# ethereum/pos-evolution

Hardware: AMD Instinct MI355X
Metric: attestations aggregated/sec + get_head() p50 latency at 1M validators (higher is better)
Workload: dtype int32

## Files before the change

include/posevo_profile.h:

```cpp
#ifndef POSEVO_PROFILE_H
#define POSEVO_PROFILE_H
#include "posevo.h"
#ifdef __cplusplus
extern "C" {
#endif

#define PE_KERNEL_G1_ACCUMULATE 0
#define PE_KERNEL_G1_NORMALISE  1
#define PE_KERNEL_VOTES         2
#define PE_KERNEL_TREE          3
#define PE_KERNEL_LMD           4
#define PE_KERNEL_PARTICIPATION 5
#define PE_KERNEL_BITS_UNION    6
#define PE_KERNEL_G2_ACCUMULATE 7
#define PE_KERNEL_G2_NORMALISE  8
#define PE_KERNEL_G1_TREE       9
#define PE_KERNEL_ATT_GROUP     10
#define PE_KERNEL_ATT_VALIDATE  11
#define PE_KERNEL_PAIR_INGEST_VALIDATE 12
#define PE_KERNEL_PAIR_PLAN_LMD        13
#define PE_KERNEL_PAIR_MEMBERS_VOTES   14
#define PE_KERNEL_PAIR_UNION_TREE      15
#define PE_KERNEL_G2_DECOMPRESS 16
#define PE_KERNEL_COUNT         17
int pe_profile_enable(pe_engine* h, int on);
int pe_profile_reset(pe_engine* h);
int pe_profile_get(pe_engine* h, int kernel, uint64_t* launches, double* total_ms);
int pe_profile_timeline(pe_engine* h, int32_t* kernel, double* start_ms, double* duration_ms, uint32_t cap, uint32_t* out_n);

int pe_profile_queue_classes(pe_engine* h, int32_t out_class[4]);
int pe_profile_arena_growths(const pe_engine* h, uint64_t* out);
int pe_profile_committee_sums(const pe_engine* h, uint32_t* out_tables_with_sums, uint32_t* out_groups_by_complement);
int pe_profile_accumulate_mhz(pe_engine* h, double* out_mhz, uint32_t cap, uint32_t* out_n);
int pe_profile_pairing_gt(pe_engine* h, const uint8_t* g1_points96, const uint8_t* g2_points192, uint64_t n_pairs,
                          const uint32_t* offsets, uint32_t n_groups, uint8_t* out576);
#define PE_BATCH_CHUNK_MAX 64
int pe_profile_batch_set_chunk(pe_engine* h, uint32_t chunk);
int pe_profile_batch_stats(const pe_engine* h, uint32_t out[8]);
int pe_profile_batch_gt(const pe_engine* h, uint8_t* out576);

#define PE_VERIFY_STRIPE_MAX 16
int pe_profile_verify_set_stripe(pe_engine* h, uint32_t k);
int pe_profile_verify_stats(const pe_engine* h, uint32_t out[5]);
int pe_profile_verify_sums(const pe_engine* h, uint32_t n_groups, uint8_t* out_pk96, uint8_t* out_sig192);

#define PE_VERIFY_RESIDENT_STATS 11
int pe_profile_verify_resident_stats(const pe_engine* h, uint32_t out[PE_VERIFY_RESIDENT_STATS]);

#ifdef __cplusplus
}
#endif
#endif
```

pos_evolution_amd/_abi.py:

```python
from __future__ import annotations

import ctypes as C
import os

_HERE = os.path.dirname(os.path.abspath(__file__))
LIB_PATH = os.environ.get("POSEVO_LIB_PATH") or os.path.join(_HERE, "libposevo.so")

PE_OK = 0
PE_ERR_NO_DEVICE = -2
PE_ERR_UNKNOWN_PARENT = -4
PE_ERR_UNKNOWN_ROOT = -9
PE_ERR_CAPACITY = -10
PE_ERR_STATE = -14
PE_ERR_TIMEOUT = -15
PE_DIST_SINGLE_COMM = 1
PE_SIG_G2_COMPRESSED, PE_SIG_G2_UNCOMPRESSED, PE_SIG_CHECK_SUBGROUP = 1, 2, 0x100
PE_SIG_STATUS_IDENTITY = 4
PE_BLS_INVALID, PE_BLS_VALID, PE_BLS_BAD_POINT, PE_BLS_UNDECIDED = 0, 1, 2, 3
PE_VERIFY_APPLY = 0x1
PE_VERIFY_RESIDENT_STATS = 11
NONE32 = 0xFFFFFFFF

PE_VAL_ACTIVE, PE_VAL_SLASHED, PE_VAL_EQUIVOCATING, PE_VAL_ACTIVE_PREV = 0x01, 0x02, 0x04, 0x08
PE_ATT_FLAG_SIGNATURE_VALID, PE_ATT_FLAG_FROM_BLOCK = 0x1, 0x2
PE_G1_PARTIAL_BYTES = 192
PE_EXCHANGE_EXTRA = 512
PE_DIST_ID_BYTES = 256
(PE_KERNEL_G1_ACCUMULATE, PE_KERNEL_G1_NORMALISE, PE_KERNEL_VOTES, PE_KERNEL_TREE, PE_KERNEL_LMD,
 PE_KERNEL_PARTICIPATION, PE_KERNEL_BITS_UNION, PE_KERNEL_G2_ACCUMULATE, PE_KERNEL_G2_NORMALISE,
 PE_KERNEL_G1_TREE, PE_KERNEL_ATT_GROUP, PE_KERNEL_ATT_VALIDATE, PE_KERNEL_PAIR_INGEST_VALIDATE,
 PE_KERNEL_PAIR_PLAN_LMD, PE_KERNEL_PAIR_MEMBERS_VOTES, PE_KERNEL_PAIR_UNION_TREE, PE_KERNEL_G2_DECOMPRESS,
 PE_KERNEL_COUNT) = range(18)
KERNEL_NAMES = ["g1_accumulate", "g1_normalise", "votes", "tree", "lmd", "participation", "bits_union",
                "g2_accumulate", "g2_normalise", "g1_tree", "att_group", "att_validate", "pair_ingest_validate",
                "pair_plan_lmd", "pair_members_votes", "pair_union_tree", "g2_decompress"]

ATT_STATUS_NAMES = {
    0: "ok", 1: "target epoch not current or previous", 2: "target epoch != epoch(slot)",
    3: "unknown target root", 4: "unknown beacon block root", 5: "block after attestation slot",
    6: "target not ancestor of beacon block", 7: "attestation slot not in the past", 8: "no committee table",
    9: "committee index out of range", 10: "bits length mismatch", 11: "empty or invalid indices",
    12: "bad signature", 13: "outside inclusion window", 14: "source mismatch",
    32: "slasher: target epoch in the future", 33: "slasher: target epoch left the window",
    34: "slasher: data table of the epoch is full",
}
PE_ATT_UNKNOWN_TARGET_ROOT, PE_ATT_UNKNOWN_BEACON_BLOCK_ROOT = 3, 4
PE_SLASH_FUTURE_TARGET, PE_SLASH_TOO_OLD, PE_SLASH_TABLE_FULL = 32, 33, 34
PE_SLASH_APPLY = 1
PE_SLASH_DOUBLE, PE_SLASH_SURROUND = 1, 2


class pe_config(C.Structure):
    _fields_ = [
        ("slots_per_epoch", C.c_uint64), ("seconds_per_slot", C.c_uint64), ("intervals_per_slot", C.c_uint64),
        ("safe_slots_to_update_justified", C.c_uint64), ("proposer_score_boost", C.c_uint64),
        ("effective_balance_increment", C.c_uint64), ("min_attestation_inclusion_delay", C.c_uint64),
        ("max_validators_per_committee", C.c_uint64), ("filter_slashed", C.c_uint32), ("device", C.c_int32),
        ("reserve_validators", C.c_uint64), ("reserve_blocks", C.c_uint32), ("max_committee_tables", C.c_uint32),
        ("vote_expiry_slots", C.c_uint64),
    ]


class pe_attestation(C.Structure):
    _fields_ = [
        ("slot", C.c_uint64), ("index", C.c_uint64), ("beacon_block_root", C.c_uint8 * 32),
        ("source_epoch", C.c_uint64), ("source_root", C.c_uint8 * 32),
        ("target_epoch", C.c_uint64), ("target_root", C.c_uint8 * 32),
        ("bits_offset", C.c_uint32), ("n_bits", C.c_uint32), ("flags", C.c_uint32), ("reserved0", C.c_uint32),
    ]


assert C.sizeof(pe_attestation) == 144


class pe_state_ctx(C.Structure):
    _fields_ = [
        ("slot", C.c_uint64), ("chain_tip_root", C.c_uint8 * 32),
        ("current_justified_epoch", C.c_uint64), ("current_justified_root", C.c_uint8 * 32),
        ("previous_justified_epoch", C.c_uint64), ("previous_justified_root", C.c_uint8 * 32),
        ("base_reward_per_increment", C.c_uint64),
    ]


class pe_prune_stats(C.Structure):
    _fields_ = [("blocks_before", C.c_uint32), ("blocks_after", C.c_uint32), ("votes_remapped", C.c_uint64),
                ("votes_orphaned", C.c_uint64)]


# ... 221 lines not shown
```

pos_evolution_amd/csrc/att_bodies.inc:

```
#include <algorithm>
#include "att_rules.h"
#include "kernels.h"
#include "wave64.h"

namespace posevo {

namespace {

constexpr uint32_t VAL_EQUIVOCATING_BIT = 0x04u;
constexpr uint32_t ERR_INVALID_ARG = 1, ERR_CAPACITY = 10, ERR_NO_COMMITTEES = 11;

struct Row9 { uint4 q[9]; };
__device__ __forceinline__ void load_row(Row9& r, const uint4* __restrict__ rows, uint32_t i)
{
    const uint4* p = rows + (size_t)9 * i;
#pragma unroll
    for (int k = 0; k < 9; ++k) r.q[k] = p[k];
}
__device__ __forceinline__ unsigned long long u64_of(uint32_t lo, uint32_t hi) { return ((unsigned long long)hi << 32) | lo; }
__device__ __forceinline__ unsigned long long row_slot(const Row9& r) { return u64_of(r.q[0].x, r.q[0].y); }
__device__ __forceinline__ unsigned long long row_index(const Row9& r) { return u64_of(r.q[0].z, r.q[0].w); }
__device__ __forceinline__ unsigned long long row_source_epoch(const Row9& r) { return u64_of(r.q[3].x, r.q[3].y); }
__device__ __forceinline__ unsigned long long row_target_epoch(const Row9& r) { return u64_of(r.q[5].z, r.q[5].w); }

// ... 424 lines not shown
    }
}
struct Root2 { uint4 lo, hi; };
struct BlockStoreDev {
    const BlockTableDev& bt;
    __device__ __forceinline__ uint32_t find(const Root2& r) const { return find_block_dev(bt, r.lo, r.hi); }
    __device__ __forceinline__ uint32_t handle(uint32_t idx) const { return bt.pos_of_idx[idx]; }
    __device__ __forceinline__ unsigned long long slot_of(uint32_t idx) const { return bt.slot_pos[bt.pos_of_idx[idx]]; }
    __device__ __forceinline__ uint32_t ancestor(uint32_t idx, unsigned long long slot) const
    {
        uint32_t p = bt.pos_of_idx[idx];
        while (bt.slot_pos[p] > slot && bt.parent_pos[p] != NONE32) p = bt.parent_pos[p];
        return p;
    }
};
}

namespace {
__device__ __forceinline__ void att_validate_fc_body(const uint32_t g , const ValidateFcArgs& a)
{
    const uint4* __restrict__ rows = static_cast<const uint4*>(a.rows);
    const AttGroup* __restrict__ grp = a.grp;
    const AttPlan* __restrict__ plan = a.plan;
    const uint32_t cap = a.cap;
    const BlockTableDev& bt = a.bt;
    const FcCtx& fc = a.fc;
    const uint32_t* __restrict__ union_info = a.union_info;
    AttRow* __restrict__ out_rows = a.out_rows;
    int32_t* __restrict__ status_dev = a.status_dev;
    int32_t* __restrict__ status_host = a.status_host;
    uint32_t* __restrict__ count_host = a.count_host;
    uint32_t* __restrict__ err_host = a.err_host;
    const uint32_t ng = plan->n_groups;
    if (ng > cap) {
        if (g < ng) status_dev[g] = -1;
        if (g == 0) *err_host = ERR_CAPACITY;
        return;
    }
    if (g >= ng) return;
    const AttGroup G = grp[g];
    Row9 r;
    load_row(r, rows, G.rep);
    const unsigned long long slot = row_slot(r), tep = row_target_epoch(r), spe = fc.slots_per_epoch;
    const FcVerdict v = att_fork_choice_status(BlockStoreDev{bt}, (r.q[8].z & FLAG_FROM_BLOCK) != 0, slot, tep, Root2{r.q[6], r.q[7]},
                                               Root2{r.q[1], r.q[2]}, fc.cur_slot, fc.cur_epoch, fc.prev_epoch, spe);
    int32_t st = v.status;
    if (st == ST_OK) st = (int32_t)G.status_agg;
    const uint32_t cnt = union_info[2 * g], overlap = union_info[2 * g + 1];
    if (st == ST_OK) st = att_indexed_status(G.sig_valid != 0, overlap != 0, cnt);
    out_rows[g] = att_row_fork_choice(G.member_base, G.size, G.out_word, v.block, tep, slot, g, g);
    status_dev[g] = st;
    status_host[g] = st;
    if (count_host) count_host[g] = st == ST_OK ? cnt : 0u;
}
}

namespace {
__device__ __forceinline__ void lmd_vm_tables_body(const unsigned long long v , const LmdVmArgs& a)
{
    const AttRow* __restrict__ rows = a.rows;
    const TablesDev& tables = a.tables;
    const uint32_t* __restrict__ cs0 = a.crow_start[0];
    const uint32_t* __restrict__ cs1 = a.crow_start[1];
    const uint32_t* __restrict__ cl0 = a.crow_list[0];
    const uint32_t* __restrict__ cl1 = a.crow_list[1];
    const AttPlan* __restrict__ plan = a.plan;
    const uint32_t* __restrict__ bit_arena = a.bit_arena;
    const uint8_t* __restrict__ flags = a.flags;
    unsigned long long* __restrict__ vote_key = reinterpret_cast<unsigned long long*>(a.vote_key);
    uint32_t* __restrict__ vote_block = a.vote_block;
    uint32_t* __restrict__ vote_slot = a.vote_slot;
    const uint32_t* __restrict__ gates = a.gates;
    if (v >= a.n_val) return;
    uint32_t best_e = 0, best_order = NONE32, new_block = NONE32, new_slot = 0;
    bool loaded = false;
    for (int t = 0; t < 2; ++t) {
        if (!tables.t[t].valid || plan->n_rows_table[t] == 0) continue;
        const uint32_t c = tables.t[t].inv_comm[v];
        if (c == NONE32) continue;
        const uint32_t* crow_start = t ? cs1 : cs0;
        const uint32_t* crow_list = t ? cl1 : cl0;
        const uint32_t kb = crow_start[c], ke = crow_start[c + 1];
        if (kb == ke) continue;
        if (!loaded) {
            if (flags[v] & VAL_EQUIVOCATING_BIT) return;
            best_e = (uint32_t)(vote_key[v] >> 32);
            loaded = true;
        }
        const uint32_t i = tables.t[t].inv_pos[v];
        for (uint32_t k = kb; k < ke; ++k) {
            const AttRow r = rows[crow_list[k]];
            if (i >= r.n_bits) continue;
            if (gates[r.gate] != 0) continue;
            if (!((bit_arena[r.bits_word + (i >> 5)] >> (i & 31)) & 1u)) continue;
            if (r.epoch_p1 > best_e || (r.epoch_p1 == best_e && new_block != NONE32 && r.order < best_order)) {
                best_e = r.epoch_p1;
                best_order = r.order;
                new_block = r.block_idx;
                new_slot = r.slot;
            }
        }
    }
    if (new_block != NONE32) {
        vote_key[v] = ((unsigned long long)best_e << 32) | 0xFFFFFFFFull;
        vote_block[v] = new_block;
        if (vote_slot) vote_slot[v] = new_slot;
    }
}
}

}
```

pos_evolution_amd/csrc/engine_g1.cpp:

```cpp
#include "engine_internal.h"

using namespace posevo;

namespace posevo {

void g1_stream_guard(pe_engine* h, hipStream_t s)
{
    if (h->side_ever && s != h->side_stream && s != h->fin_stream && s != h->norm_stream) (void)hipStreamWaitEvent(s, h->ev_join, 0);
}

int build_points30(pe_engine* h, uint64_t n)
{
    HIP_TRY(h, h->d_points30.ensure(std::max<size_t>(128, 4ull * G1_ROW_WORDS * n)));
    launch_g1_table_s30(h->stream, h->d_points.as<uint32_t>(), h->d_points30.as<uint32_t>(), n);
    HIP_TRY(h, hipGetLastError());
    h->points30_valid = true;
    return PE_OK;
}

int launch_g1_planned(pe_engine* h, const uint32_t* d_points, const uint32_t* d_members, const uint32_t* d_bits,
                      const G1Group* d_groups, const G1Plan& plan, uint8_t* d_out96, uint32_t* dev_jac,
                      hipStream_t s, hipStream_t fin, DevBuf* partials, DevBuf* lane_partials, const AttPlan* plan_dev,
                      const uint32_t* d_members1, uint64_t caller_rows, const G1Complement* cm)
{
    if (plan.n_groups == 0) return PE_OK;
    if (!s) s = h->stream;
    if (!fin) fin = s;
    if (!partials) partials = &h->d_partials;
    if (!lane_partials) lane_partials = &h->d_lane_partials;
    PE_TRY(ensure_quiesced(h, *partials,
                           std::max<size_t>(PE_G1_PARTIAL_BYTES, (size_t)PE_G1_PARTIAL_BYTES * plan.n_partials)));
    const size_t lane_bytes = (size_t)G1_LANE_PARTIAL_BYTES * G1_WG * ((plan.n_slots + G1_WG - 1) / G1_WG);
    PE_TRY(ensure_quiesced(h, *lane_partials, std::max<size_t>(PE_G1_PARTIAL_BYTES, lane_bytes)));
    const uint32_t* d_points30;
    if (d_points == h->d_points.as<uint32_t>()) {
        if (!h->points30_valid) return fail(h, PE_ERR_STATE, "the registry's table of the accumulation's field form was not built");
        d_points30 = h->d_points30.as<uint32_t>();
    } else {
        const uint64_t n_rows = caller_rows;
        if (d_points != h->d_tmp_points.as<uint32_t>() || 4ull * G1_ROW_WORDS * n_rows > h->d_tmp_points.cap)
            return fail(h, PE_ERR_STATE, "G1 sum over an unknown point table");
        HIP_TRY(h, h->d_tmp_points30.ensure(std::max<size_t>(128, 4ull * G1_ROW_WORDS * n_rows)));
        launch_g1_table_s30(s, d_points, h->d_tmp_points30.as<uint32_t>(), n_rows);
        d_points30 = h->d_tmp_points30.as<uint32_t>();
    }
    const bool chain = fin != s && fin == h->fin_stream;
    const int exclusive = chain && h->tune.exclusive && h->blocks.size() <= 4096 ? 1 : 0;
    const uint32_t sparse_max = cm && cm->info ? h->tune.g1_sparse_max() : 0u;
    const uint32_t* sparse_info = sparse_max ? cm->info : nullptr;
    if (sparse_max)
        launch_g1_absentees(s, d_points30, d_members, d_members1, d_bits, d_groups, plan.n_groups, plan_dev, cm->cmpl, sparse_info,
                            sparse_max, partials->as<uint32_t>());
    {
        const bool skip = !h->prof_timeline && s != h->stream && (h->acc_launches++ & 3) != 0;
        ProfScope ps(h, PE_KERNEL_G1_ACCUMULATE, s, skip);
        unsigned long long* clock_rec = nullptr;
        if (h->profiling) {
            if (!h->acc_clock && hipHostMalloc(reinterpret_cast<void**>(&h->acc_clock), 16ull * pe_engine::ACC_CLOCK_RING,
                                               hipHostMallocDefault) != hipSuccess) {
                (void)hipGetLastError();
                h->acc_clock = nullptr;
            }
            if (h->acc_clock) {
                clock_rec = h->acc_clock + 2 * (h->acc_clock_n++ % pe_engine::ACC_CLOCK_RING);
                clock_rec[0] = clock_rec[1] = 0;
            }
        }
        launch_g1_accumulate(s, d_points30, d_members, d_bits, d_groups, plan.n_groups, plan.n_slots,
                             lane_partials->as<uint32_t>(), partials->as<uint32_t>(), plan_dev, d_members1, exclusive, clock_rec,
                             cm ? cm->cmpl : nullptr, sparse_info, sparse_max);
    }
    hipStream_t ts = fin;
    if (ts != s) {
        HIP_TRY(h, hipEventRecord(h->ev_acc, s));
        HIP_TRY(h, hipStreamWaitEvent(ts, h->ev_acc, 0));
    }
    {
        ProfScope ps(h, PE_KERNEL_G1_TREE, ts);
        launch_g1_tree(ts, lane_partials->as<uint32_t>(), d_groups, plan.n_groups, plan.n_slots, partials->as<uint32_t>(),
                       ts != s ? 1 : 0,
                       plan_dev, exclusive, sparse_max ? cm->cmpl : nullptr, sparse_info, sparse_max);
    }
    hipStream_t ns = fin;
    if (chain && h->norm_stream) {
        ns = h->norm_stream;
        HIP_TRY(h, hipEventRecord(h->ev_tree, ts));
        HIP_TRY(h, hipStreamWaitEvent(ns, h->ev_tree, 0));
    } else if (ts != fin) {
        HIP_TRY(h, hipEventRecord(h->ev_tree, ts));
        HIP_TRY(h, hipStreamWaitEvent(fin, h->ev_tree, 0));
    }
    if (cm)
        for (int t = 0; t < 2; ++t)
            if (cm->ev[t]) HIP_TRY(h, hipStreamWaitEvent(ns, cm->ev[t], 0));
    {
        ProfScope ps(h, PE_KERNEL_G1_NORMALISE, ns);
        launch_g1_finish(ns, partials->as<uint32_t>(), d_groups, plan.n_groups, 0, 0, d_out96, dev_jac, plan_dev,
                         cm ? cm->cmpl : nullptr, cm ? cm->sums[0] : nullptr, cm ? cm->sums[1] : nullptr);
    }
    HIP_TRY(h, hipGetLastError());
    return PE_OK;
}

void committee_sums_drop(pe_engine* h)
{
// ... 690 lines not shown
```

pos_evolution_amd/csrc/engine_internal.h:

```cpp
#pragma once
#include <hip/hip_runtime.h>
#include <dlfcn.h>
#include <rccl/rccl.h>

#include <algorithm>
#include <array>
#include <chrono>
#include <cstdlib>
#include <map>
#include <cstdio>
#include <cstddef>
#include <cstring>
#include <functional>
#include <memory>
#include <new>
#include <numeric>
#include <string>
#include <thread>
#include <unordered_map>
#include <vector>

#include "../../include/posevo.h"
#include "../../include/posevo_profile.h"
#include "att_rules.h"
// ... 223 lines not shown
    DevBuf d_vote_slot;
    DevBuf d_sbalance, d_sflags;
    bool state_view_set = false;
    std::vector<uint8_t> h_flags;
    DevBuf d_activation_epoch, d_exit_epoch;
    bool epochs_set = false;
    DevBuf d_active, d_active_wg;
    bool active_valid = false;
    uint64_t active_epoch = 0;
    uint32_t active_n = 0;
    hipEvent_t ev_active_read = nullptr;
    bool active_read_pending = false;
    DevBuf d_rbalance, d_inactivity, d_withdrawable;
    bool balances_set = false;
    DevBuf d_registry_wg;
    DevBuf d_pubkey_leaf, d_withdrawal_credentials, d_activation_eligibility;
    bool static_set = false;
    DevBuf d_ssz_zero;
    bool ssz_zero_ready = false;
    DevBuf d_ssz_validator_roots;
    DevBuf d_ssz_level[2];
    DevBuf d_ssz_chunks;
    DevBuf d_bls;
    struct ResidentVerify {
        bool valid = false;
        uint64_t rr_generation = 0, res_generation = 0;
        int arena = 0;
        uint32_t n_in = 0;
        bool checked_subgroup = false;
    } rv;
    uint32_t* keep_pk = nullptr;
    std::vector<uint8_t> verify_head;
    uint32_t verify_resident_stats[PE_VERIFY_RESIDENT_STATS] = {};
    DevBuf d_batch;
    uint32_t batch_chunk = 2;
    uint32_t batch_stats[8] = {};
    uint8_t batch_gt[576] = {};
    DevBuf d_verify;
    uint32_t verify_stripe = 16;
    uint32_t verify_stats[5] = {};
    std::vector<uint8_t> verify_sums_pk, verify_sums_sig;

    bool tree_dirty = true;
    DevBuf d_tsize, d_tparent, d_trank, d_tleaf, d_tpos, d_tidx, d_direct, d_weights, d_totals, d_head;
    DevBuf d_broot_tab, d_broots, d_bslot_pos;
    uint32_t broot_mask = 0;
    std::vector<uint32_t> h_pos_of_idx;
    PinBuf h_head;
    uint32_t votes_grid = 0;
    bool weights_stale = false;

    std::vector<CommitteeTable> tables;
    uint64_t table_stamp = 0;
    size_t last_table = 0;

    DevBuf d_partials, d_lane_partials, d_out96, d_tmp_points, d_tmp_be;

    struct PipeArena {
        DevBuf d_stage, d_outblk;
        PinBuf h_stage, h_pin;
        DevBuf d_res_bits, d_res_info;
        DevBuf d_partials, d_lane_partials;
        DevBuf d_rr_tab, d_rr;
        DevBuf d_sig_in, d_sig_pts, d_sig_status;
        DevBuf d_res_points;
        uint32_t rr_rows_cap = 0, rr_comm_cap = 0, rr_tab_size = 0;
        DevBuf x_rr_tab, x_rr, x_res_bits, x_res_info;
        uint32_t x_rows_cap = 0, x_comm_cap = 0, x_tab_size = 0;
        DevBuf d_xsend, d_xrecv, d_xrows, d_xbits, d_xn;
        size_t stage_cursor = 0, out_cursor = 0;
        uint64_t table_stamp_at_begin = 0;
        uint64_t generation = 0;
        std::vector<std::function<int()>> pending;
        hipEvent_t ev_main = nullptr, ev_side = nullptr, ev_aux = nullptr;
        hipEvent_t ev_leg = nullptr;
        bool leg_used = false;
        bool fenced = false, side_used = false, aux_used = false;
        bool fence_pending = false;
        bool aux_reads_scratch = false;
    };
    static constexpr int MAX_ARENAS = 16;
    int n_arenas = 3;
    PipeArena arena[MAX_ARENAS];
    int cur = 0;
    PipeArena& A() { return arena[cur]; }
    bool pipelining = false;
    uint64_t pipes_begun = 0, pipes_completed = 0;
    hipStream_t side_stream = nullptr;
    uint64_t arena_growths = 0;
    bool queues_distinct = false;
    hipStream_t fin_stream = nullptr;
    hipStream_t norm_stream = nullptr;
    hipEvent_t ev_tree = nullptr;
    hipStream_t g1_tail() const { return norm_stream ? norm_stream : fin_stream; }
    hipStream_t aux_stream = nullptr;
    hipStream_t aux_owned = nullptr;
    hipStream_t prep_stream = nullptr;
    DevBuf d_shuffle_scratch;
    hipStream_t sums_stream = nullptr;
    DevBuf d_sum_groups, d_sum_lane;
    uint32_t last_cmpl_groups = 0;
    hipEvent_t ev_aux_fork = nullptr;
    hipEvent_t ev_aux_switch = nullptr;
    static constexpr uint32_t STATE_ON_SIDE_MAX_ROWS = 1024;
    bool aux_busy = false;
    bool state_work_on_main = false;
    hipEvent_t ev_acc = nullptr;
    struct SigSeg {
        int arena;
        uint32_t n;
        bool compressed, check_subgroup;
        bool streaming;
        const uint8_t* d_in;
        const uint8_t* copy_from;
        size_t bytes;
        uint32_t* d_pts; int32_t* d_status;
        const UnionGroup* d_ug; const uint32_t* d_member_row; uint32_t ng_bound; const AttPlan* plan_dev;
        uint8_t* o_sig; uint32_t* o_bad; int32_t* o_st;
        uint32_t* keep_mont48; uint32_t* keep_bad;
    };
    std::vector<SigSeg> sig_batch;
    hipEvent_t ev_sig = nullptr;
    hipEvent_t ev_fork = nullptr, ev_join = nullptr;
    bool side_busy = false;
    bool side_ever = false;
    bool streaming = false;
    std::vector<std::function<int()>> deferred;
    struct HeldFc {
        bool active = false;
        int arena = -1;
        bool have_fc = false;
        bool have_head = false;
        ValidateFcArgs validate{};
        LmdVmArgs lmd{};
        VotesArgs votes{};
        TreeArgs tree{};
        std::function<int()> between;
        std::vector<std::function<int()>> g1;
        bool fence_pending = false;
    } held;
    bool pairing = std::getenv("POSEVO_PAIR") == nullptr || std::atoi(std::getenv("POSEVO_PAIR")) != 0;
    struct Tune {
        static int env(const char* name, int dflt)
        {
            const char* e = std::getenv(name);
            return e && *e ? std::atoi(e) : dflt;
        }
        int exclusive = env("POSEVO_ACC_EXCLUSIVE", 1);
        int state_on = env("POSEVO_STATE_ON", 2);
        int sig_batch = env("POSEVO_SIG_BATCH", 8);
        int queue_probe = env("POSEVO_QUEUE_PROBE", 1);
        int committee_sums = env("POSEVO_COMMITTEE_SUMS", 1);
        int g1_sparse = env("POSEVO_G1_SPARSE", 1);
        uint32_t g1_sparse_max() const
        {
            return g1_sparse <= 0 ? 0u : g1_sparse == 1 ? G1_SPARSE_MAX : std::min<uint32_t>((uint32_t)g1_sparse, G1_SPARSE_CAP);
        }
        uint32_t ssz_tile_log2 = (uint32_t)std::min<int>(SSZ_TILE_LOG2, std::max<int>(SSZ_TILE_LOG2_MIN, env("POSEVO_SSZ_TILE_LOG2", SSZ_TILE_LOG2)));
    } tune;

    struct ResGroup { uint32_t byte_off, n_bits, word, sig_valid, tag; };
    std::vector<ResGroup> res_groups;
    std::shared_ptr<std::vector<uint32_t>> res_info_host;
    bool res_valid = false;
    int res_arena = 0;
    uint64_t res_generation = 0;

    struct ResidentRows {
        bool valid = false;
        int arena = 0;
        uint32_t n_in = 0;
        const void* rows = nullptr;
        TablesDev tables{};
        uint64_t generation = 0;
        int set = 0;
        uint32_t n_groups = 0;
    } rr;

    int g1_tune_calls = 0;
    float g1_tune_best[2] = {1e30f, 1e30f};
    uint32_t g1_target_slots = 0;
    hipEvent_t g1_tune_ev[2] = {nullptr, nullptr};
    bool points30_valid = false;
    DevBuf d_points30, d_tmp_points30;

    ncclComm_t comm = nullptr, comm_g1 = nullptr;
    int early_rc = PE_OK;
    uint32_t xchg_blocks = 0;
    uint64_t xchg_nval = 0;
    bool last_agg_on_side = false;
    int dist_rank = 0, dist_world = 1;
    DevBuf d_xchg, d_xpart, d_xgather;
    pe_collectives coll{};
    bool coll_custom = false;
    bool dist_single_comm = false;
    bool dist_wedged = false;
    uint32_t dist_timeout_ms = 30000;
    uint32_t dist_max_groups = 0;
    hipEvent_t ev_xchg = nullptr;
    bool dist_ready() const { return comm != nullptr || coll_custom; }

    struct Slasher {
        bool enabled = false;
        uint32_t history = 0, max_data = 0;
        uint64_t n_val = 0;
        bool have_window = false;
        uint64_t window = 0;
        DevBuf d_rec, d_ids, d_counter, d_evidence;
        struct EpochData {
            std::vector<std::array<uint8_t, 128>> data;
// ... 2 lines not shown
        std::vector<EpochData> epochs;
        bool on_device = false;
        uint32_t tab_size = 0;
        DevBuf d_data, d_count, d_tab;
        DevBuf d_work;
        std::vector<uint32_t> dev_count;
    } slasher;

    bool profiling = false;
    uint64_t acc_launches = 0;
    static constexpr uint32_t ACC_CLOCK_RING = 4096;
    unsigned long long* acc_clock = nullptr;
    uint64_t acc_clock_n = 0;
    KernelProfile prof[PE_KERNEL_COUNT];
    bool prof_timeline = false;
    bool prof_dominant_only = false;
    hipEvent_t prof_base = nullptr;
    struct TimelineEntry { int32_t kernel; float start_ms, dur_ms; };
    std::vector<TimelineEntry> prof_tl;
    std::vector<hipEvent_t> event_pool;
    HostTrace trace;
};

namespace posevo {

int fail(pe_engine* h, int code, const std::string& msg);
int hip_fail(pe_engine* h, hipError_t e, const char* what);
#define HIP_TRY(h, expr)                                        \
    do {                                                        \
        hipError_t _e = (expr);                                 \
        if (_e != hipSuccess) return hip_fail((h), _e, #expr);  \
    } while (0)
#define PE_TRY(expr)              \
    do {                          \
        const int _rc = (expr);   \
        if (_rc) return _rc;      \
    } while (0)

struct ProfScope {
    pe_engine* h;
    int k;
    hipStream_t s;
    hipEvent_t a = nullptr, b = nullptr;
    static hipEvent_t take(pe_engine* h)
    {
        if (!h->event_pool.empty()) { hipEvent_t e = h->event_pool.back(); h->event_pool.pop_back(); return e; }
        hipEvent_t e = nullptr;
        return hipEventCreate(&e) == hipSuccess ? e : nullptr;
    }
    ProfScope(pe_engine* h_, int k_, hipStream_t s_ = nullptr, bool sampled_out = false) : h(h_), k(k_), s(s_ ? s_ : h_->stream)
    {
        if (!h->profiling || sampled_out) return;
        if (h->prof_dominant_only && k != PE_KERNEL_G1_ACCUMULATE) return;
        if ((k == PE_KERNEL_ATT_GROUP || k == PE_KERNEL_ATT_VALIDATE) && !h->prof_timeline) return;
        a = take(h);
        b = take(h);
        if (!a || !b) { a = b = nullptr; return; }
        (void)hipEventRecord(a, s);
    }
    ~ProfScope()
    {
        if (!a) return;
        (void)hipEventRecord(b, s);
        h->prof[k].pending.emplace_back(a, b);
    }
};

int run_deferred(pe_engine* h);
int complete_arena(pe_engine* h, int ai);
void complete_oldest_if_ready(pe_engine* h);
int flush_pending(pe_engine* h);
int enter(pe_engine* h);
extern const uint8_t NEG_G1_BE96[96];
int draw_scalars(pe_engine* h, std::vector<uint64_t>& out);
int pairing_run(pe_engine* h, const char* who, const uint8_t* g1, const uint8_t* g2, uint64_t n_pairs, const uint32_t* offsets,
                uint32_t n_groups, int32_t* verdict, uint8_t* out576);
using WireAt = std::function<const uint8_t*(uint32_t)>;
int verify_pairs_run(pe_engine* h, const char* who, uint32_t n, const WireAt& pk_at, const WireAt& msg_at, const WireAt& sig_at,
                     int32_t* verdict);
struct ResPoints { uint32_t *pk_xyzz48, *sig_mont48, *sig_bad; size_t bytes; };
inline ResPoints res_points_layout(void* base, uint32_t n)
{
    const size_t rows = std::max<uint32_t>(n, 1);
    Layout l;
    const auto pk = l.take<uint32_t>(48 * rows), sig = l.take<uint32_t>(48 * rows), bad = l.take<uint32_t>(rows);
    return ResPoints{pk.at(base), sig.at(base), bad.at(base), l.total()};
}
inline int refuse_dist(pe_engine* h, const char* who)
{
    return fail(h, PE_ERR_STATE, std::string(who) + ": the handle exchanges with other ranks (pe_dist_init); "
                                                    "the sharded handles are not supported");
}
int need_init(pe_engine* h, bool flush = true, bool keep_held = false);
bool hold_eligible(const pe_engine* h);
int held_issue(pe_engine* h);
int launch_rows_paired(pe_engine* h, const IngestArgs& ia, const AttPlanArgs& pa, const MembersArgs& ma, const UnionArgs& ua);
int fence_arena(pe_engine* h, pe_engine::PipeArena& a);
int tree_args(pe_engine* h, uint64_t* d_direct, const VoteTotals* d_totals, int clear_direct, uint32_t* head_word, TreeArgs* out);
VotesArgs votes_args(const pe_engine* h);
hipStream_t state_stream_begin(pe_engine* h, bool reads_scratch = false, uint32_t rows_hint = 0);
hipStream_t leg_stream(pe_engine* h);
bool probe_queue_classes(const std::vector<hipStream_t>& streams, std::vector<int>& cls);
int sig_batch_flush(pe_engine* h);
bool sig_batch_holds(const pe_engine* h, int arena);
hipStream_t state_stream_unordered(pe_engine* h);
int aux_join(pe_engine* h, hipStream_t ms);

// ... 336 lines not shown
```

pos_evolution_amd/csrc/engine_resident.cpp:

```cpp
#include "engine_internal.h"


using namespace posevo;

namespace posevo {

namespace {

struct RrLayout {
    AttPlan* plan;
    uint32_t *slot_of, *rep_of, *gid_of_row, *ubytes, *member_row;
    PlanSync* sync;
    PlanRec* rec;
    AttGroup* grp;
    UnionGroup* ug;
    G1Group* g1;
    AttRow *rows_fc, *rows_st;
    int32_t *status_fc, *status_st;
    uint32_t* cmpl;
    uint32_t *crow_start[2], *crow_cursor[2], *crow_cnt[2], *crow_list[2];
    size_t bytes;
};

RrLayout rr_layout(uint8_t* base, uint32_t cap_n, uint32_t cap_c)
{
    RrLayout L;
    size_t off = 0;
    auto take = [&](size_t bytes) {
        uint8_t* p = base ? base + off : nullptr;
        off = (off + bytes + 255) & ~size_t(255);
        return p;
    };
    L.plan = reinterpret_cast<AttPlan*>(take(sizeof(AttPlan)));
    L.slot_of = reinterpret_cast<uint32_t*>(take(4ull * cap_n));
    L.rep_of = reinterpret_cast<uint32_t*>(take(4ull * cap_n));
    L.gid_of_row = reinterpret_cast<uint32_t*>(take(4ull * cap_n));
    L.sync = reinterpret_cast<PlanSync*>(take(sizeof(PlanSync)));
    L.rec = reinterpret_cast<PlanRec*>(take(sizeof(PlanRec) * ((size_t)cap_n / PLAN_WG + 1)));
    L.ubytes = reinterpret_cast<uint32_t*>(take(4ull * cap_n));
    L.member_row = reinterpret_cast<uint32_t*>(take(4ull * cap_n));
    L.grp = reinterpret_cast<AttGroup*>(take(sizeof(AttGroup) * (size_t)cap_n));
    L.ug = reinterpret_cast<UnionGroup*>(take(sizeof(UnionGroup) * (size_t)cap_n));
    L.g1 = reinterpret_cast<G1Group*>(take(sizeof(G1Group) * (size_t)cap_n));
    L.rows_fc = reinterpret_cast<AttRow*>(take(sizeof(AttRow) * (size_t)cap_n));
    L.rows_st = reinterpret_cast<AttRow*>(take(sizeof(AttRow) * (size_t)cap_n));
    L.status_fc = reinterpret_cast<int32_t*>(take(4ull * cap_n));
    L.status_st = reinterpret_cast<int32_t*>(take(4ull * cap_n));
    L.cmpl = reinterpret_cast<uint32_t*>(take(4ull * cap_n));
    for (int t = 0; t < 2; ++t) {
        L.crow_start[t] = reinterpret_cast<uint32_t*>(take(4ull * (cap_c + 1)));
        L.crow_cursor[t] = reinterpret_cast<uint32_t*>(take(4ull * (cap_c + 1)));
        L.crow_cnt[t] = reinterpret_cast<uint32_t*>(take(4ull * (cap_c + 1)));
        L.crow_list[t] = reinterpret_cast<uint32_t*>(take(4ull * cap_n));
    }
    L.bytes = off;
    return L;
}

struct RrSet {
    DevBuf &tab, &rr, &bits, &info;
    uint32_t &rows_cap, &comm_cap, &tab_size;
};
RrSet rr_set(pe_engine::PipeArena& a, int set)
{
    if (set == 0) return RrSet{a.d_rr_tab, a.d_rr, a.d_res_bits, a.d_res_info, a.rr_rows_cap, a.rr_comm_cap, a.rr_tab_size};
    return RrSet{a.x_rr_tab, a.x_rr, a.x_res_bits, a.x_res_info, a.x_rows_cap, a.x_comm_cap, a.x_tab_size};
}
RrLayout rr_of(pe_engine::PipeArena& a, int set = 0)
{
    const RrSet s = rr_set(a, set);
    return rr_layout(s.rr.as<uint8_t>(), s.rows_cap, s.comm_cap);
}

int rr_ensure(pe_engine* h, pe_engine::PipeArena& arena, int set, uint32_t n, uint32_t n_comm)
{
    {
        const RrSet rs = rr_set(arena, set);
        if (n <= rs.rows_cap && n_comm <= rs.comm_cap && rs.rr.p && rs.tab.p) return PE_OK;
    }
    PE_TRY(flush_pending(h));
    HIP_TRY(h, hipDeviceSynchronize());
    uint32_t cap_n = 1024, cap_c = 64;
    for (int i = 0; i < h->n_arenas; ++i) {
        const RrSet o = rr_set(h->arena[i], set);
        cap_n = std::max(cap_n, o.rows_cap);
        cap_c = std::max(cap_c, o.comm_cap);
    }
    while (cap_n < n) cap_n *= 2;
    while (cap_c < n_comm) cap_c *= 2;
    uint32_t tab = 2048;
    while (tab < 2 * cap_n) tab <<= 1;
    const RrLayout L = rr_layout(nullptr, cap_n, cap_c);
    for (int i = 0; i < h->n_arenas; ++i) {
        pe_engine::PipeArena& other = h->arena[i];
        if (set != 0 && &other != &arena) continue;
        const RrSet a = rr_set(other, set);
        if (cap_n <= a.rows_cap && cap_c <= a.comm_cap && a.rr.p && a.tab.p) continue;
        a.rr.release();
        a.tab.release();
        HIP_TRY(h, a.rr.ensure(L.bytes));
        HIP_TRY(h, a.tab.ensure(8ull * tab));
        HIP_TRY(h, hipMemsetAsync(a.tab.p, 0xFF, 4ull * tab, h->stream));
        HIP_TRY(h, hipMemsetAsync(a.tab.as<uint8_t>() + 4ull * tab, 0, 4ull * tab, h->stream));
        HIP_TRY(h, hipMemsetAsync(a.rr.p, 0, L.bytes, h->stream));
        a.rows_cap = cap_n;
        a.comm_cap = cap_c;
// ... 325 lines not shown
    out->res_bits = RS.bits.as<uint32_t>();
    out->res_info = RS.info.as<uint32_t>();
    out->n_in = h->rr.n_in;
    return PE_OK;
}

int resident_lists(pe_engine* h, const UnionGroup** ug, const uint32_t** member_row)
{
    if (!h->rr.valid) return fail(h, PE_ERR_STATE, "no aggregate over rows in device memory on this handle");
    const RrLayout L = rr_of(h->arena[h->rr.arena], h->rr.set);
    *ug = L.ug;
    *member_row = L.member_row;
    return PE_OK;
}

int resident_precheck(pe_engine* h, const char* who)
{
    if (!h->rr.valid) return fail(h, PE_ERR_STATE, std::string(who) + ": PE_ROWS_RESIDENT without a pe_aggregate over rows in device memory on this handle");
    TablesDev now;
    CommitteeTable* tabs[2];
    PE_TRY(candidate_tables(h, &now, tabs));
    for (int t = 0; t < 2; ++t)
        if (now.t[t].epoch != h->rr.tables.t[t].epoch || now.t[t].valid != h->rr.tables.t[t].valid ||
            now.t[t].members != h->rr.tables.t[t].members)
            return fail(h, PE_ERR_STATE, std::string(who) + ": the store's clock or its committee tables changed since the resident pe_aggregate: aggregate again");
    return PE_OK;
}

int on_attestation_resident(pe_engine* h, uint32_t cap, int32_t* status, uint32_t* out_count)
{
    PE_TRY(resident_precheck(h, "pe_on_attestation_batch"));
    if (cap == 0) return PE_OK;
    if (h->held.active && (h->held.arena != h->cur || h->held.have_fc || h->held.have_head)) PE_TRY(held_issue(h));
    HostLap lap(&h->trace);
    PE_TRY(refresh_tree(h));
    pe_engine::PipeArena& RA = h->arena[h->rr.arena];
    const RrLayout L = rr_of(RA, h->rr.set);
    const RrSet RS = rr_set(RA, h->rr.set);
    Stage st(h);
    OutBlock ob(h);
    const size_t off_status = ob.alloc(4ull * cap);
    const size_t off_count = ob.alloc(4ull * cap);
    const size_t off_err = ob.alloc(16);
    PE_TRY(ob.ensure());
    *ob.host<uint32_t>(off_err) = 0;
    FcCtx fc;
    fc.cur_slot = current_slot(h);
    fc.cur_epoch = epoch_at_slot(h, fc.cur_slot);
    fc.prev_epoch = fc.cur_epoch > 0 ? fc.cur_epoch - 1 : 0;
    fc.slots_per_epoch = h->cfg.slots_per_epoch;
    const uint32_t n_launch = std::max<uint32_t>(h->rr.n_in, 1);
    memset(ob.host<int32_t>(off_status), 0, 4ull * cap);
    memset(ob.host<uint32_t>(off_count), 0, 4ull * cap);
    const ValidateFcArgs va{h->rr.rows, L.grp, L.plan, n_launch, cap, block_table_dev(h), fc, RS.info.as<uint32_t>(), L.rows_fc,
                            L.status_fc, ob.host<int32_t>(off_status), ob.host<uint32_t>(off_count), ob.host<uint32_t>(off_err)};
    const LmdVmArgs la{L.rows_fc, h->rr.tables, {L.crow_start[0], L.crow_start[1]}, {L.crow_list[0], L.crow_list[1]}, L.plan,
                       RS.bits.as<uint32_t>(), h->d_flags.as<uint8_t>(), h->n_val, h->d_vote_key.as<uint64_t>(),
                       h->d_vote_block.as<uint32_t>(), h->cfg.vote_expiry_slots ? h->d_vote_slot.as<uint32_t>() : nullptr,
                       reinterpret_cast<const uint32_t*>(L.status_fc)};
    if (hold_eligible(h) && h->rr.arena == h->cur && h->rr.set == 0 && h->n_val) {
        h->held.validate = va;
        h->held.lmd = la;
        h->held.have_fc = true;
        h->held.active = true;
        h->held.arena = h->cur;
    } else {
        if (h->held.active) PE_TRY(held_issue(h));
        {
            ProfScope ps(h, PE_KERNEL_ATT_VALIDATE);
            launch_att_validate_fc(h->stream, va);
        }
        ProfScope ps(h, PE_KERNEL_LMD);
        launch_lmd_vm_tables(h->stream, la);
    }
    HIP_TRY(h, hipGetLastError());
    lap.mark("ratt.1_launch");
    const size_t base = ob.base;
    const int ai = h->cur;
    auto complete = [h, ai, base, off_status, off_count, off_err, cap, status, out_count]() -> int {
        const uint8_t* pin = h->arena[ai].h_pin.as<uint8_t>() + base;
        const uint32_t err = *reinterpret_cast<const uint32_t*>(pin + off_err);
        if (err) return plan_error_to_status(h, err, "pe_on_attestation_batch (PE_ROWS_RESIDENT)");
        memcpy(status, pin + off_status, 4ull * cap);
        if (out_count) memcpy(out_count, pin + off_count, 4ull * cap);
        return PE_OK;
    };
    HostLap lap2(&h->trace);
    const int rc = finish_call(h, st, ob, complete);
    lap2.mark("ratt.2_wait_outputs");
    return rc;
}

int process_attestation_resident(pe_engine* h, const pe_state_ctx* sc, uint32_t cap, int32_t* status, uint64_t* out_numerators)
{
    PE_TRY(resident_precheck(h, "pe_process_attestation_batch"));
    if (cap == 0) return PE_OK;
    const uint64_t spe = h->cfg.slots_per_epoch;
    if (spe > 64) return fail(h, PE_ERR_CAPACITY, "PE_ROWS_RESIDENT: SLOTS_PER_EPOCH above 64");
    uint32_t tip;
    if (!find_block(h, to_root(sc->chain_tip_root), &tip)) return fail(h, PE_ERR_UNKNOWN_ROOT, "chain tip unknown");
    HostLap lap(&h->trace);
    PE_TRY(refresh_tree(h));
    pe_engine::PipeArena& RA = h->arena[h->rr.arena];
    const RrLayout L = rr_of(RA, h->rr.set);
    const RrSet RS = rr_set(RA, h->rr.set);
    Stage st(h);
    StateCtxDev S;
    memset(&S, 0, sizeof(S));
    S.slot = sc->slot;
    S.cur_epoch = sc->slot / spe;
    S.prev_epoch = S.cur_epoch > 0 ? S.cur_epoch - 1 : 0;
    S.slots_per_epoch = spe;
// ... 60 lines not shown
```

pos_evolution_amd/csrc/kernels.h:

```cpp
#pragma once
#include <hip/hip_runtime.h>
#include <stdint.h>

namespace posevo {

template <int TAG>
static bool first_use_on_this_device()
{
    static bool done[64] = {false};
    int dev = 0;
    (void)hipGetDevice(&dev);
    if (dev < 0 || dev >= 64) return true;
    if (done[dev]) return false;
    done[dev] = true;
    return true;
}

constexpr uint32_t NONE32 = 0xFFFFFFFFu;
constexpr int G1_ROW_WORDS = 32;
constexpr int G2_WG_SLOTS = 128;
constexpr int G1_WG = 256;
constexpr int G1_LANE_PARTIAL_BYTES = 208;
constexpr int TREE_MAX_BLOCKS = 8192;
constexpr int VOTES_MAX_WG = 256;
// ... 147 lines not shown
    uint32_t tgt_blk[2];
    uint32_t head_blk[64];
    unsigned long long base_reward_per_increment;
};
struct PlanSync {
    uint32_t ticket;
    uint32_t max_size;
    uint32_t rows_t[2];
    uint32_t mis_key;
    uint32_t err;
    uint32_t pad[2];
    unsigned long long total_members, pad2[3];
};
struct PlanRec {
    unsigned long long agg[3], incl[3], pad[2];
};
constexpr uint32_t PLAN_WG = 256;
constexpr uint32_t PLAN_MAX_ROWS = 1u << 24;
struct AttPlanArgs {
    const void* rows; uint32_t n; const uint32_t* n_dev;
    const uint32_t* tab; const uint32_t* cnt_tab; const uint32_t* slot_of;
    uint32_t* rep_of; uint32_t* gid_of_row;
    AttGroup* grp; UnionGroup* ug;
    uint32_t* crow_start[2]; uint32_t* crow_cursor[2]; uint32_t* crow_cnt[2];
    PlanSync* sync; PlanRec* rec;
    AttPlan* plan; AttPlan* plan_host;
    uint64_t out_arena_cap; uint32_t target_slots, slot_cap, min_k, want_pk;
    TablesDev tables;
};
void launch_att_plan(hipStream_t s, const AttPlanArgs& a);
void launch_att_pack(hipStream_t s, const void* rows, const AttGroup* grp, const AttPlan* plan, const uint32_t* res_bits,
                     const uint32_t* res_info, uint32_t slots, uint32_t wps, uint32_t* send);
void launch_att_unpack(hipStream_t s, const uint32_t* recv, uint32_t world, uint32_t slots, uint32_t wps, void* out_rows,
                       uint32_t* out_bits, uint32_t* n_dev, uint32_t* err_host);
void launch_att_validate_state(hipStream_t s, const void* rows, const AttGroup* grp, const AttPlan* plan, uint32_t n_bound,
                               uint32_t cap, BlockTableDev bt, const StateCtxDev& st, const uint32_t* union_info,
                               AttRow* out_rows, int32_t* status_dev, int32_t* status_host, uint32_t* err_host);
void launch_participation_tables(hipStream_t s, const AttRow* rows, TablesDev tables, uint32_t* const crow_start[2],
                                 uint32_t* const crow_list[2], const AttPlan* plan, const uint32_t* bit_arena,
                                 const uint16_t* eff_increments, uint64_t base_reward_per_increment,
                                 uint32_t* part_cur_words, uint32_t* part_prev_words, uint64_t* numerators,
                                 const uint32_t* gates, uint32_t cap);

struct IngestArgs {
    const void* rows; uint32_t n;
    uint32_t* tab; uint32_t* cnt_tab;
    uint32_t tab_mask;
    uint32_t* slot_of;
    uint64_t arena_len; AttPlan* plan;
    void* arena_pad32;
    const uint32_t* n_dev;
    const void* arena_src; void* arena_dst;
};
struct ValidateFcArgs {
    const void* rows; const AttGroup* grp; const AttPlan* plan;
    uint32_t n_bound, cap;
    BlockTableDev bt; FcCtx fc;
    const uint32_t* union_info; AttRow* out_rows; int32_t* status_dev; int32_t* status_host; uint32_t* count_host;
    uint32_t* err_host;
};
struct LmdVmArgs {
    const AttRow* rows; TablesDev tables; const uint32_t* crow_start[2]; const uint32_t* crow_list[2];
    const AttPlan* plan; const uint32_t* bit_arena; const uint8_t* flags; uint64_t n_val; uint64_t* vote_key;
    uint32_t* vote_block; uint32_t* vote_slot; const uint32_t* gates;
};
struct MembersArgs {
    const void* rows; uint32_t n; uint32_t* tab; uint32_t* cnt_tab; const uint32_t* slot_of; const uint32_t* rep_of;
    const uint32_t* gid_of_row; AttGroup* grp; AttPlan* plan; uint32_t* ubytes; uint32_t* member_row;
    uint32_t* host_group_of; void* host_out_rows; const uint32_t* n_dev;
    G1Group* g1; uint32_t* crow_cursor[2]; uint32_t* crow_list[2];
};
struct VotesArgs {
    const uint32_t* vote_block; const uint64_t* eff_balance; const uint8_t* flags; uint64_t n_val;
    uint32_t filter_slashed; const uint32_t* pos_of_idx; uint32_t n_blocks; uint64_t* direct; VoteTotals* totals;
    const uint32_t* vote_slot; uint32_t min_vote_slot;
};
struct UnionArgs {
    const UnionGroup* groups; uint32_t n_groups; const uint32_t* att_bytes;
    const uint8_t* bit_arena;
    uint32_t* out_arena;
    uint32_t* out_info;
    uint32_t* host_arena; uint32_t* host_info;
    const AttPlan* plan_dev;
    uint32_t* cmpl; uint32_t* host_cmpl; const AttGroup* grp; uint32_t sums_ok[2];
};
struct TreeArgs {
    TreeDev tree; uint64_t* direct; const VoteTotals* totals; uint64_t ov_balance, ov_num; int use_override;
    uint32_t justified_pos, boost_pos; uint64_t slots_per_epoch, boost_percent, balance_increment;
    uint64_t* weights_by_idx; uint32_t* head_idx; int clear_direct;
};
struct RemapArgs {
    uint32_t* vote_block; uint64_t n_val;
    const uint32_t* map; uint32_t n_old;
    unsigned long long* counts;
};
constexpr uint32_t VOTE_PRUNED = 0xFFFFFFFEu;
constexpr int REMAP_WG = 256;
constexpr unsigned REMAP_MAX_WG = 256;
void launch_votes_remap(hipStream_t s, const RemapArgs& a);
void launch_att_ingest(hipStream_t s, const IngestArgs& a);
void launch_att_validate_fc(hipStream_t s, const ValidateFcArgs& a);
void launch_lmd_vm_tables(hipStream_t s, const LmdVmArgs& a);
void launch_att_members(hipStream_t s, const MembersArgs& a);
void launch_votes(hipStream_t s, const VotesArgs& a, int lean);
void votes_clear_exchange(hipStream_t s, uint64_t* direct, uint32_t n_blocks, VoteTotals* totals);
void launch_bits_union(hipStream_t s, const UnionArgs& a);
void launch_tree(hipStream_t s, const TreeArgs& a, int lean);
bool launch_pair_ingest_validate(hipStream_t s, const IngestArgs& rows_next, const ValidateFcArgs& fc_prev);
bool launch_pair_plan_lmd(hipStream_t s, const AttPlanArgs& rows_next, const LmdVmArgs& fc_prev);
bool launch_pair_members_votes(hipStream_t s, const MembersArgs& rows_next, const VotesArgs& fc_prev);
bool launch_pair_union_tree(hipStream_t s, const UnionArgs& rows_next, const TreeArgs& fc_prev);
void pair_kernels_preload();

struct SlashRow {
    uint32_t bits_byte;
    uint32_t n_bits;
    uint32_t source, target;
// ... 242 lines not shown
```

Baseline: 5.938 billion.

## Precompute per-committee LMD records in validate to skip CSR walks for singletons

The validate kernel now writes a compact 32-byte record per committee position holding the attestation's bits offset, block, epoch, order and slot, plus a stamp and a kind tag (single accepted, single rejected, multi). The LMD vote kernel reads this record first: it skips rejected singletons outright and handles accepted singletons with one bit test, instead of walking crow_start and crow_list and loading full AttRow entries. The goal is fewer dependent global loads per validator in the hot LMD pass. The cost is extra writes and arena space in validate, and a per-call serial stamp to invalidate stale records. It also adds a profiling slot for the g1 absentees kernel.

```diff
diff --git a/include/posevo_profile.h b/include/posevo_profile.h
--- a/include/posevo_profile.h
+++ b/include/posevo_profile.h
@@ -22,7 +22,8 @@
 #define PE_KERNEL_PAIR_MEMBERS_VOTES   14
 #define PE_KERNEL_PAIR_UNION_TREE      15
 #define PE_KERNEL_G2_DECOMPRESS 16
-#define PE_KERNEL_COUNT         17
+#define PE_KERNEL_G1_ABSENTEES  17
+#define PE_KERNEL_COUNT         18
 int pe_profile_enable(pe_engine* h, int on);
 int pe_profile_reset(pe_engine* h);
 int pe_profile_get(pe_engine* h, int kernel, uint64_t* launches, double* total_ms);
diff --git a/pos_evolution_amd/_abi.py b/pos_evolution_amd/_abi.py
--- a/pos_evolution_amd/_abi.py
+++ b/pos_evolution_amd/_abi.py
@@ -30,10 +30,10 @@
  PE_KERNEL_PARTICIPATION, PE_KERNEL_BITS_UNION, PE_KERNEL_G2_ACCUMULATE, PE_KERNEL_G2_NORMALISE,
  PE_KERNEL_G1_TREE, PE_KERNEL_ATT_GROUP, PE_KERNEL_ATT_VALIDATE, PE_KERNEL_PAIR_INGEST_VALIDATE,
  PE_KERNEL_PAIR_PLAN_LMD, PE_KERNEL_PAIR_MEMBERS_VOTES, PE_KERNEL_PAIR_UNION_TREE, PE_KERNEL_G2_DECOMPRESS,
- PE_KERNEL_COUNT) = range(18)
+ PE_KERNEL_G1_ABSENTEES, PE_KERNEL_COUNT) = range(19)
 KERNEL_NAMES = ["g1_accumulate", "g1_normalise", "votes", "tree", "lmd", "participation", "bits_union",
                 "g2_accumulate", "g2_normalise", "g1_tree", "att_group", "att_validate", "pair_ingest_validate",
-                "pair_plan_lmd", "pair_members_votes", "pair_union_tree", "g2_decompress"]
+                "pair_plan_lmd", "pair_members_votes", "pair_union_tree", "g2_decompress", "g1_absentees"]
 
 ATT_STATUS_NAMES = {
     0: "ok", 1: "target epoch not current or previous", 2: "target epoch != epoch(slot)",
diff --git a/pos_evolution_amd/csrc/att_bodies.inc b/pos_evolution_amd/csrc/att_bodies.inc
--- a/pos_evolution_amd/csrc/att_bodies.inc
+++ b/pos_evolution_amd/csrc/att_bodies.inc
@@ -500,6 +500,17 @@
     status_dev[g] = st;
     status_host[g] = st;
     if (count_host) count_host[g] = st == ST_OK ? cnt : 0u;
+    if (a.lmd_rec[0] && G.table != NONE32 && G.status_agg == (uint32_t)ST_OK) {
+        const uint32_t* __restrict__ cs = a.crow_start[G.table];
+        LmdRec* rec = a.lmd_rec[G.table] + G.pos;
+        if (cs[G.pos + 1] - cs[G.pos] == 1u) {
+            uint4* q = reinterpret_cast<uint4*>(rec);
+            q[0] = make_uint4(G.size, G.out_word, v.block, (uint32_t)tep + 1u);
+            q[1] = make_uint4(g, (uint32_t)slot, a.lmd_stamp, st == ST_OK ? LMD_REC_SINGLE_OK : LMD_REC_SINGLE_REJECTED);
+        } else {
+            *reinterpret_cast<uint2*>(&rec->stamp) = make_uint2(a.lmd_stamp, LMD_REC_MULTI);
+        }
+    }
 }
 }
 
@@ -519,6 +530,8 @@
     uint32_t* __restrict__ vote_block = a.vote_block;
     uint32_t* __restrict__ vote_slot = a.vote_slot;
     const uint32_t* __restrict__ gates = a.gates;
+    const LmdRec* __restrict__ rec0 = a.lmd_rec[0];
+    const LmdRec* __restrict__ rec1 = a.lmd_rec[1];
     if (v >= a.n_val) return;
     uint32_t best_e = 0, best_order = NONE32, new_block = NONE32, new_slot = 0;
     bool loaded = false;
@@ -528,14 +541,39 @@
         if (c == NONE32) continue;
         const uint32_t* crow_start = t ? cs1 : cs0;
         const uint32_t* crow_list = t ? cl1 : cl0;
-        const uint32_t kb = crow_start[c], ke = crow_start[c + 1];
-        if (kb == ke) continue;
+        const LmdRec* __restrict__ recs = t ? rec1 : rec0;
+        uint4 q0 = make_uint4(0u, 0u, 0u, 0u), q1 = q0;
+        bool single = false;
+        if (recs) {
+            const uint4* q = reinterpret_cast<const uint4*>(recs + c);
+            q0 = q[0];
+            q1 = q[1];
+            if (q1.z != a.lmd_stamp || q1.w == LMD_REC_SINGLE_REJECTED) continue;
+            single = q1.w == LMD_REC_SINGLE_OK;
+        }
+        uint32_t kb = 0, ke = 0;
+        if (!single) {
+            kb = crow_start[c];
+            ke = crow_start[c + 1];
+            if (kb == ke) continue;
+        }
         if (!loaded) {
             if (flags[v] & VAL_EQUIVOCATING_BIT) return;
             best_e = (uint32_t)(vote_key[v] >> 32);
             loaded = true;
         }
         const uint32_t i = tables.t[t].inv_pos[v];
+        if (single) {
+            if (i >= q0.x) continue;
+            if (!((bit_arena[q0.y + (i >> 5)] >> (i & 31)) & 1u)) continue;
+            if (q0.w > best_e || (q0.w == best_e && new_block != NONE32 && q1.x < best_order)) {
+                best_e = q0.w;
+                best_order = q1.x;
+                new_block = q0.z;
+                new_slot = q1.y;
+            }
+            continue;
+        }
         for (uint32_t k = kb; k < ke; ++k) {
             const AttRow r = rows[crow_list[k]];
             if (i >= r.n_bits) continue;
diff --git a/pos_evolution_amd/csrc/engine_g1.cpp b/pos_evolution_amd/csrc/engine_g1.cpp
--- a/pos_evolution_amd/csrc/engine_g1.cpp
+++ b/pos_evolution_amd/csrc/engine_g1.cpp
@@ -48,9 +48,11 @@
     const int exclusive = chain && h->tune.exclusive && h->blocks.size() <= 4096 ? 1 : 0;
     const uint32_t sparse_max = cm && cm->info ? h->tune.g1_sparse_max() : 0u;
     const uint32_t* sparse_info = sparse_max ? cm->info : nullptr;
-    if (sparse_max)
+    if (sparse_max) {
+        ProfScope ps(h, PE_KERNEL_G1_ABSENTEES, s);
         launch_g1_absentees(s, d_points30, d_members, d_members1, d_bits, d_groups, plan.n_groups, plan_dev, cm->cmpl, sparse_info,
                             sparse_max, partials->as<uint32_t>());
+    }
     {
         const bool skip = !h->prof_timeline && s != h->stream && (h->acc_launches++ & 3) != 0;
         ProfScope ps(h, PE_KERNEL_G1_ACCUMULATE, s, skip);
diff --git a/pos_evolution_amd/csrc/engine_internal.h b/pos_evolution_amd/csrc/engine_internal.h
--- a/pos_evolution_amd/csrc/engine_internal.h
+++ b/pos_evolution_amd/csrc/engine_internal.h
@@ -299,6 +299,7 @@
 
     std::vector<CommitteeTable> tables;
     uint64_t table_stamp = 0;
+    uint32_t lmd_serial = 0;
     size_t last_table = 0;
 
     DevBuf d_partials, d_lane_partials, d_out96, d_tmp_points, d_tmp_be;
@@ -403,6 +404,7 @@
         {
             return g1_sparse <= 0 ? 0u : g1_sparse == 1 ? G1_SPARSE_MAX : std::min<uint32_t>((uint32_t)g1_sparse, G1_SPARSE_CAP);
         }
+        int lmd_rec = env("POSEVO_LMD_REC", 1);
         uint32_t ssz_tile_log2 = (uint32_t)std::min<int>(SSZ_TILE_LOG2, std::max<int>(SSZ_TILE_LOG2_MIN, env("POSEVO_SSZ_TILE_LOG2", SSZ_TILE_LOG2)));
     } tune;
 
@@ -511,7 +513,7 @@
     {
         if (!h->profiling || sampled_out) return;
         if (h->prof_dominant_only && k != PE_KERNEL_G1_ACCUMULATE) return;
-        if ((k == PE_KERNEL_ATT_GROUP || k == PE_KERNEL_ATT_VALIDATE) && !h->prof_timeline) return;
+        if ((k == PE_KERNEL_ATT_GROUP || k == PE_KERNEL_ATT_VALIDATE || k == PE_KERNEL_G1_ABSENTEES) && !h->prof_timeline) return;
         a = take(h);
         b = take(h);
         if (!a || !b) { a = b = nullptr; return; }
diff --git a/pos_evolution_amd/csrc/engine_resident.cpp b/pos_evolution_amd/csrc/engine_resident.cpp
--- a/pos_evolution_amd/csrc/engine_resident.cpp
+++ b/pos_evolution_amd/csrc/engine_resident.cpp
@@ -19,6 +19,7 @@
     int32_t *status_fc, *status_st;
     uint32_t* cmpl;
     uint32_t *crow_start[2], *crow_cursor[2], *crow_cnt[2], *crow_list[2];
+    LmdRec* lmd_rec[2];
     size_t bytes;
 };
 
@@ -52,6 +53,7 @@
         L.crow_cursor[t] = reinterpret_cast<uint32_t*>(take(4ull * (cap_c + 1)));
         L.crow_cnt[t] = reinterpret_cast<uint32_t*>(take(4ull * (cap_c + 1)));
         L.crow_list[t] = reinterpret_cast<uint32_t*>(take(4ull * cap_n));
+        L.lmd_rec[t] = reinterpret_cast<LmdRec*>(take(sizeof(LmdRec) * ((size_t)cap_c + 1)));
     }
     L.bytes = off;
     return L;
@@ -483,12 +485,18 @@
     const uint32_t n_launch = std::max<uint32_t>(h->rr.n_in, 1);
     memset(ob.host<int32_t>(off_status), 0, 4ull * cap);
     memset(ob.host<uint32_t>(off_count), 0, 4ull * cap);
+    const bool lmd_rec = h->tune.lmd_rec != 0;
+    if (lmd_rec && ++h->lmd_serial == 0) ++h->lmd_serial;
+    const uint32_t stamp = lmd_rec ? h->lmd_serial : 0u;
+    LmdRec* const rec0 = lmd_rec ? L.lmd_rec[0] : nullptr;
+    LmdRec* const rec1 = lmd_rec ? L.lmd_rec[1] : nullptr;
     const ValidateFcArgs va{h->rr.rows, L.grp, L.plan, n_launch, cap, block_table_dev(h), fc, RS.info.as<uint32_t>(), L.rows_fc,
-                            L.status_fc, ob.host<int32_t>(off_status), ob.host<uint32_t>(off_count), ob.host<uint32_t>(off_err)};
+                            L.status_fc, ob.host<int32_t>(off_status), ob.host<uint32_t>(off_count), ob.host<uint32_t>(off_err),
+                            {rec0, rec1}, {L.crow_start[0], L.crow_start[1]}, stamp};
     const LmdVmArgs la{L.rows_fc, h->rr.tables, {L.crow_start[0], L.crow_start[1]}, {L.crow_list[0], L.crow_list[1]}, L.plan,
                        RS.bits.as<uint32_t>(), h->d_flags.as<uint8_t>(), h->n_val, h->d_vote_key.as<uint64_t>(),
                        h->d_vote_block.as<uint32_t>(), h->cfg.vote_expiry_slots ? h->d_vote_slot.as<uint32_t>() : nullptr,
-                       reinterpret_cast<const uint32_t*>(L.status_fc)};
+                       reinterpret_cast<const uint32_t*>(L.status_fc), {rec0, rec1}, stamp};
     if (hold_eligible(h) && h->rr.arena == h->cur && h->rr.set == 0 && h->n_val) {
         h->held.validate = va;
         h->held.lmd = la;
diff --git a/pos_evolution_amd/csrc/kernels.h b/pos_evolution_amd/csrc/kernels.h
--- a/pos_evolution_amd/csrc/kernels.h
+++ b/pos_evolution_amd/csrc/kernels.h
@@ -223,17 +223,26 @@
     const uint32_t* n_dev;
     const void* arena_src; void* arena_dst;
 };
+struct alignas(32) LmdRec {
+    uint32_t n_bits, bits_word, block_idx, epoch_p1;
+    uint32_t order, slot;
+    uint32_t stamp;
+    uint32_t kind;
+};
+constexpr uint32_t LMD_REC_SINGLE_OK = 1, LMD_REC_SINGLE_REJECTED = 2, LMD_REC_MULTI = 3;
 struct ValidateFcArgs {
     const void* rows; const AttGroup* grp; const AttPlan* plan;
     uint32_t n_bound, cap;
     BlockTableDev bt; FcCtx fc;
     const uint32_t* union_info; AttRow* out_rows; int32_t* status_dev; int32_t* status_host; uint32_t* count_host;
     uint32_t* err_host;
+    LmdRec* lmd_rec[2]; const uint32_t* crow_start[2]; uint32_t lmd_stamp;
 };
 struct LmdVmArgs {
     const AttRow* rows; TablesDev tables; const uint32_t* crow_start[2]; const uint32_t* crow_list[2];
     const AttPlan* plan; const uint32_t* bit_arena; const uint8_t* flags; uint64_t n_val; uint64_t* vote_key;
     uint32_t* vote_block; uint32_t* vote_slot; const uint32_t* gates;
+    const LmdRec* lmd_rec[2]; uint32_t lmd_stamp;
 };
 struct MembersArgs {
     const void* rows; uint32_t n; uint32_t* tab; uint32_t* cnt_tab; const uint32_t* slot_of; const uint32_t* rep_of;
```

Measured after the change: 5.497 billion. 0.926x the previous value.
